# lyclyc52/Instance_NeRF

Measured on AMD Instinct MI355X. Metric: Msamples/sec (train+infer) 3D-FRONT 800x800 at 1/2/4/8 MI355X; PSNR parity, higher is better.
Workload: dtype f32; 1 GPU; render 800x800 synthetic 3D-FRONT-like room, hash-grid NeRF L=16 F=2 T=6119864 sigma+rgb (BASELINE configs[1]), one view per step per GPU; parallelism=views sharded over 1 GPU(s), no data-path collective

## Files before the change

### instance_nerf_amd/csrc/field_fused.hip

```cpp
#include <atomic>
#include <mutex>
#include <type_traits>

#include "common.h"
#include "grid_common.h"
#include "sample_pos.h"

namespace inr {

typedef float f32x4 __attribute__((ext_vector_type(4)));
typedef __bf16 bf16x8 __attribute__((ext_vector_type(8)));

#ifndef INR_MLP_FP32
#define INR_MLP_FP32 0
#endif

#ifdef INR_PROBE_BUILD
#include "probe/field_probe.h"
#else
#if defined(INR_PROBE_MODE) || defined(INR_PROBE_STATIC) || defined(INR_PROBE_SLOW_XCD)
#error "INR_PROBE_* switches need -DINR_PROBE_BUILD (tools/build_probe.py): those variants produce wrong results"
#endif
#define INR_PROBE_PROLOGUE()
#define INR_PROBE_SCHEDULE(steal)
// ... 362 lines not shown
__device__ __forceinline__ uint32_t pack_f16x2(float a, float b) {
  const f32x2_t v = {a, b};
  return __builtin_bit_cast(uint32_t, __builtin_convertvector(v, f16x2_t));
}
template <int N_MT, int N_S>
__device__ __forceinline__ void layer_h1(const uint4* __restrict__ w, int lane, const uint4* in, f32x4* out) {
  f32x4 acc[N_MT];
#pragma unroll
  for (int mt = 0; mt < N_MT; ++mt) acc[mt] = f32x4{0.f, 0.f, 0.f, 0.f};
#pragma unroll
  for (int st = 0; st < N_S; ++st) {
    __builtin_amdgcn_sched_barrier(0);
#pragma unroll
    for (int mt = 0; mt < N_MT; ++mt)
      acc[mt] = __builtin_amdgcn_mfma_f32_16x16x32_f16(__builtin_bit_cast(f16x8_t, w[((mt * N_S + st) * 2 + 0) * 64 + lane]),
                                                       __builtin_bit_cast(f16x8_t, in[st]), acc[mt], 0, 0, 0);
  }
#pragma unroll
  for (int mt = 0; mt < N_MT; ++mt) out[mt] = acc[mt];
}

template <int N_MT, int N_G, bool kFast = false>
__device__ __forceinline__ void mlp_layer(const float4* __restrict__ wsec, int lane, const f32x4* in, f32x4* out) {
#if INR_MLP_FP32
  layer<N_MT, N_G>(wsec, lane, in, out);
#else
  if constexpr (kFast) {
    uint4 b[N_G / 2];
#pragma unroll
    for (int st = 0; st < N_G / 2; ++st)
      b[st] = uint4{pack_f16x2(in[2 * st][0], in[2 * st][1]), pack_f16x2(in[2 * st][2], in[2 * st][3]),
                    pack_f16x2(in[2 * st + 1][0], in[2 * st + 1][1]), pack_f16x2(in[2 * st + 1][2], in[2 * st + 1][3])};
    layer_h1<N_MT, N_G / 2>(reinterpret_cast<const uint4*>(wsec), lane, b, out);
  } else {
    SplitB b[N_G / 2];
#pragma unroll
    for (int st = 0; st < N_G / 2; ++st) b[st] = split8(in[2 * st], in[2 * st + 1]);
    layer_bf<N_MT, N_G / 2>(reinterpret_cast<const uint4*>(wsec), lane, b, out);
  }
#endif
}

__device__ __forceinline__ float rgb_channel_of_lane(const f32x4 o) {
  const auto a = __builtin_amdgcn_permlane16_swap(__float_as_uint(o[0]), __float_as_uint(o[1]), false, false);
  const unsigned a0 = a[0];
  const auto b = __builtin_amdgcn_permlane32_swap(a0, __float_as_uint(o[2]), false, false);
  const unsigned b0 = b[0];
  return __uint_as_float(b0);
}
__device__ __forceinline__ float sigmoid_rgb(float o) {
  return __frcp_rn(1.0f + __expf(-o));
}

__device__ __forceinline__ float select4(int q, float a, float b, float c, float d) {
  return q == 0 ? a : (q == 1 ? b : (q == 2 ? c : d));
}

struct TileIn {
  float x0, x1, x2;
  float d0, d1, d2;
  bool oob;
};

__device__ __forceinline__ float to_x01(float x, float bound, float rb, float) { return (x + bound) / rb; }

template <bool kDir>
__device__ __forceinline__ void load_tile_in(const float* __restrict__ x, const float* __restrict__ d, int64_t m,
                                             float bound, float rb, float rb_inv, TileIn& t) {
  t.x0 = to_x01(x[m * 3 + 0], bound, rb, rb_inv);
  t.x1 = to_x01(x[m * 3 + 1], bound, rb, rb_inv);
  t.x2 = to_x01(x[m * 3 + 2], bound, rb, rb_inv);
  t.oob = oob01(t.x0, t.x1, t.x2);
  if (t.oob) t.x0 = t.x1 = t.x2 = 0.0f;
  if constexpr (kDir) {
    t.d0 = d[m * 3]; t.d1 = d[m * 3 + 1]; t.d2 = d[m * 3 + 2];
  }
}

constexpr int kXcdChunkLog2 = 10;
#ifndef INR_STEAL_SHIFT
#define INR_STEAL_SHIFT 1
#endif
constexpr int kStealRoundsShift = INR_STEAL_SHIFT;
struct TileSched {
  int64_t lo, hi;
  int64_t first;
  int64_t stride;
  int64_t main_local = 0, tail_base = 0;
  int64_t n_main = 0, tail = 0;
  int64_t static_local = 0;
  uint32_t xcd = 0;
  bool interleaved = false, hybrid = false;
  __device__ __forceinline__ int64_t tile_of(int y, int64_t u) const {
    if (u < main_local) return ((((u >> kXcdChunkLog2) << 3) + y) << kXcdChunkLog2) + (u & ((1 << kXcdChunkLog2) - 1));
    return n_main + tail * y / 8 + (u - main_local);
  }
  __device__ __forceinline__ int64_t local_end(int y) const { return main_local + tail * (y + 1) / 8 - tail * y / 8; }
  __device__ __forceinline__ int64_t tile(int64_t i) const {
    if (interleaved) {
      const int64_t u = first + i * stride;
      if (u < main_local)
        return ((((u >> kXcdChunkLog2) << 3) + xcd) << kXcdChunkLog2) + (u & ((1 << kXcdChunkLog2) - 1));
      return tail_base + (u - main_local);
    }
    return first + i * stride;
  }
};
__device__ __forceinline__ TileSched make_sched(int64_t n_tiles, int waves_per_block, bool steal = false) {
  const int nb = gridDim.x, b = blockIdx.x;
  const int w = threadIdx.x >> 6;
  TileSched s;
  if (nb % 8 == 0) {
    const int xcd = b & 7, local = b >> 3, per = nb >> 3;
    const int64_t rounds = n_tiles >> (kXcdChunkLog2 + 3);
    if (rounds >= 4) {
      const int64_t n_main = rounds << (kXcdChunkLog2 + 3), tail = n_tiles - n_main;
      s.interleaved = true;
      s.xcd = (uint32_t)xcd;
      s.main_local = rounds << kXcdChunkLog2;
      s.n_main = n_main;
      s.tail = tail;
      s.hybrid = steal;
      s.static_local = steal ? (rounds - max((int64_t)1, rounds >> kStealRoundsShift)) << kXcdChunkLog2 : s.main_local;
      s.tail_base = n_main + tail * xcd / 8;
      s.lo = 0;
      s.hi = n_main + tail * (xcd + 1) / 8;
      s.first = (int64_t)local * waves_per_block + w;
      s.stride = (int64_t)per * waves_per_block;
      return s;
    }
    s.lo = n_tiles * xcd / 8;
    s.hi = n_tiles * (xcd + 1) / 8;
    s.first = s.lo + (int64_t)local * waves_per_block + w;
    s.stride = (int64_t)per * waves_per_block;
  } else {
    s.lo = 0;
    s.hi = n_tiles;
    s.first = (int64_t)b * waves_per_block + w;
    s.stride = (int64_t)nb * waves_per_block;
  }
  return s;
}

constexpr int kFieldThreads = 512;
constexpr int kGroupChunkLog2 = 6;
constexpr int kGroupDraw = 1;
constexpr int kGroupPools = 4;
struct GroupDraw {
  unsigned long long* cursor;
  int owner, n_owner;
  __device__ __forceinline__ void init(unsigned long long* cursors, int pools) {
    const int n_xcd = (gridDim.x % 8 == 0) ? 8 : 1;
    const int n_pool = (gridDim.x % (8 * pools) == 0) ? pools : 1;
    const int xcd = (n_xcd == 8) ? (int)(blockIdx.x & 7) : 0;
    const int pool = (n_pool > 1) ? (int)((blockIdx.x >> 3) % pools) : 0;
    owner = pool * n_xcd + xcd;
    n_owner = n_pool * n_xcd;
    cursor = cursors + owner;
  }
  __device__ __forceinline__ int64_t group_of(uint32_t u) const {
    const int64_t chunk = (int64_t)(u >> kGroupChunkLog2) * n_owner + owner;
    return (chunk << kGroupChunkLog2) + (u & ((1u << kGroupChunkLog2) - 1u));
  }
  __device__ __forceinline__ int64_t draw() const { return group_of((uint32_t)atomicAdd(cursor, (unsigned long long)kGroupDraw)); }
};
constexpr int kStealPools = 4, kStealOwners = 8 * kStealPools, kStealDraw = 4, kStealBlockLog2 = 6;
struct TileWalk {
  TileSched s;
  unsigned long long* cur;
  int lane, own, owner, sub;
  int64_t it, k_base;
  unsigned long long raw_next;
  bool dyn;
  __device__ __forceinline__ void init(const TileSched& sched, unsigned long long* cursors) {
    s = sched; cur = cursors; lane = threadIdx.x & 63; it = 0; dyn = false; sub = kStealDraw; k_base = 0; raw_next = 0;
    own = owner = (int)(((blockIdx.x >> 3) % kStealPools) * 8 + (blockIdx.x & 7));
    if (!cursors) s.hybrid = false;
    if (!s.hybrid) s.static_local = s.main_local;
  }
  __device__ __forceinline__ int64_t pool_len(int o) const {
    const int64_t nb = (s.local_end(o & 7) - s.static_local + (1 << kStealBlockLog2) - 1) >> kStealBlockLog2;
    const int p = o >> 3;
    return nb > p ? ((nb - p + kStealPools - 1) / kStealPools) << kStealBlockLog2 : 0;
  }
  __device__ __forceinline__ int64_t local_of(int o, int64_t k) const {
    return s.static_local + ((((k >> kStealBlockLog2) * kStealPools) + (o >> 3)) << kStealBlockLog2) +
           (k & ((1 << kStealBlockLog2) - 1));
  }
  __device__ __forceinline__ unsigned long long issue(int o) const {
    unsigned long long v = 0;
    if (lane == 0) v = atomicAdd(cur + o, (unsigned long long)kStealDraw);
    return v;
  }
  __device__ __forceinline__ static int64_t uniform(unsigned long long v) {
    return (int64_t)(((unsigned long long)(uint32_t)__builtin_amdgcn_readfirstlane((int)(v >> 32)) << 32) |
                     (uint32_t)__builtin_amdgcn_readfirstlane((int)v));
  }
  __device__ __forceinline__ int scan() const {
    bool live = false;
    if (lane < kStealOwners) live = (int64_t)__hip_atomic_load(cur + lane, __ATOMIC_RELAXED, __HIP_MEMORY_SCOPE_AGENT) < pool_len(lane);
    const uint32_t mask = (uint32_t)__ballot(live);
    for (int i = 0; i < kStealOwners; ++i) {
      const int o = (((own >> 3) + i) % kStealPools) * 8 + (((own & 7) + i / kStealPools) & 7);
      if ((mask >> o) & 1u) return o;
    }
    return -1;
  }
  __device__ __forceinline__ int64_t next() {
    if (!dyn) {
      if (!s.hybrid) {
        const int64_t t = s.tile(it++);
        return t < s.hi ? t : -1;
      }
      const int64_t u = s.first + (it++) * s.stride;
      if (u < s.static_local) return s.tile_of((int)s.xcd, u);
      dyn = true;
      raw_next = issue(owner);
    }
    for (;;) {
      if (sub < kStealDraw) {
        const int64_t u = local_of(owner, k_base + sub);
        ++sub;
        if (u < s.local_end(owner & 7)) return s.tile_of(owner & 7, u);
        continue;
      }
      int64_t k = uniform(raw_next);
      while (k >= pool_len(owner)) {
        const int o = scan();
        if (o < 0) return -1;
        owner = o;
        k = uniform(issue(owner));
      }
      k_base = k;
      sub = 0;
      raw_next = issue(owner);
    }
  }
};
constexpr int kFieldMinWaves = 2;

__device__ __forceinline__ f32x4 load4(const float* p) {
  const float4 v = *reinterpret_cast<const float4*>(p);
  return f32x4{v.x, v.y, v.z, v.w};
}
__device__ __forceinline__ void store4(float* p, f32x4 v) {
  *reinterpret_cast<float4*>(p) = make_float4(v[0], v[1], v[2], v[3]);
}
__device__ __forceinline__ f32x4 mask4(f32x4 g, f32x4 h) {
  return f32x4{h[0] > 0.f ? g[0] : 0.f, h[1] > 0.f ? g[1] : 0.f, h[2] > 0.f ? g[2] : 0.f, h[3] > 0.f ? g[3] : 0.f};
}

struct NerfSave {
  float *enc, *h1, *so, *cin, *c1, *c2;
};

constexpr int kRayRowVec = INR_RAY_TABLE_FLOATS / 4;
template <bool kColor, bool kTable = false, int kSave = 0, bool kHalf = false, bool kFast = false, bool kPre = false,
          bool kRec = false>
__global__ void __launch_bounds__(kFieldThreads, kFieldMinWaves) k_nerf_fwd(const float* __restrict__ x, const float* __restrict__ d,
                                                               int64_t M, const int32_t* __restrict__ n_dev, float bound,
                                                               const float2* __restrict__ emb, uint32_t emb_bytes, GridDesc G,
                                                               const float4* __restrict__ packed, float density_scale,
                                                               float* __restrict__ sigma, float* __restrict__ rgb,
                                                               float* __restrict__ geo, const int32_t* __restrict__ ray_ids,
                                                               const float4* __restrict__ shq, NerfSave sv,
                                                               unsigned long long* __restrict__ steal) {
  extern __shared__ __attribute__((aligned(16))) float4 wl[];
  INR_PROBE_PROLOGUE();
  __builtin_amdgcn_s_setprio(3);
  constexpr int kStage = (kColor ? kNerfFloats : kCol0) / 4;
  for (int i = threadIdx.x; i < kStage; i += kFieldThreads) wl[i] = packed[i];
  LevelRec* recs = reinterpret_cast<LevelRec*>(wl + kStage);
  stage_level_recs(G, recs);
  __syncthreads();

  constexpr int kWaves = kFieldThreads / 64;
  const int lane = threadIdx.x & 63, q = lane >> 4, j = lane & 15;
  int64_t n = M;
  if (n_dev) n = min((int64_t)*n_dev, M);
  const int64_t n_tiles = (n + 15) >> 4;
  const float rb = 2.0f * bound;
  const float rb_inv = 0.0f;
  INR_PROBE_SCHEDULE(steal);
  TileWalk walk;
  walk.init(make_sched(n_tiles, kWaves, steal != nullptr), steal);

  const bool all_hashed[4] = {slot_all_hashed(G, 0), slot_all_hashed(G, 1), slot_all_hashed(G, 2), slot_all_hashed(G, 3)};
  const __amdgpu_buffer_rsrc_t rsrc = __builtin_amdgcn_make_buffer_rsrc((void*)emb, 0, (int)emb_bytes, 0x00020000);

  for (int64_t tile = walk.next(); tile >= 0; tile = walk.next()) {
    INR_PROBE_TILE();
    const int64_t m = tile * 16 + j;
    const bool valid = m < n;
    TileIn me;
    f32x4 sh_in = {0.f, 0.f, 0.f, 0.f};
    if constexpr (kRec) {
      static_assert(!kRec || (kTable && !kPre), "the records feed is a variant of the fused table feed");
      const int64_t mm = valid ? m : n - 1;
      const float t = x[mm];
      const float4* row = shq + (int64_t)ray_ids[mm] * kRayRowVec;
      const float4 t4 = row[q], o4 = row[4], d4 = row[5];
      sh_in = f32x4{t4.x, t4.y, t4.z, t4.w};
      const float rb_rcp = 1.0f / rb;
      me.x0 = sample_x01_pow2(sample_pos(o4.x, t, d4.x, bound), bound, rb_rcp);
      me.x1 = sample_x01_pow2(sample_pos(o4.y, t, d4.y, bound), bound, rb_rcp);
      me.x2 = sample_x01_pow2(sample_pos(o4.z, t, d4.z, bound), bound, rb_rcp);
    } else if constexpr (kTable) {
      const int64_t mm = valid ? m : n - 1;
      me.x0 = x[mm * 3 + 0]; me.x1 = x[mm * 3 + 1]; me.x2 = x[mm * 3 + 2];
      const float4 t4 = shq[(int64_t)ray_ids[mm] * 4 + q];
      sh_in = f32x4{t4.x, t4.y, t4.z, t4.w};
    } else {
      load_tile_in<kColor>(x, d, valid ? m : n - 1, bound, rb, rb_inv, me);
    }

    f32x4 enc[2];
    {
      Gathered g;
      uint32_t rec_off = (uint32_t)q * 4u * (uint32_t)sizeof(LevelRec);
      asm volatile("" : "+v"(rec_off));
      typedef float v2f __attribute__((ext_vector_type(2)));
// ... 9 lines not shown
      }
      issue_gathers<kHalf, kPre>(reinterpret_cast<const LevelRec*>(reinterpret_cast<const char*>(recs) + rec_off), all_hashed,
                                 rsrc, me.x0, me.x1, me.x2, g);
      __builtin_amdgcn_sched_barrier(0);
      blend<kHalf>(g, enc[0], enc[1]);
      if constexpr (kPre) {
        if (q == 2) enc[1] = f32x4{enc[1][0], enc[1][1], fine_a.x, fine_a.y};
        else if (q == 3) enc[1] = f32x4{fine_a.x, fine_a.y, fine_b.x, fine_b.y};
      }
    }
    if constexpr (!kTable) {
      if (me.oob) enc[0] = enc[1] = f32x4{0.f, 0.f, 0.f, 0.f};
    }
    INR_PROBE_AFTER_GATHER();

    f32x4 h1[4];
    mlp_layer<4, 2, kFast>(wl + kSig0 / 4, lane, enc, h1);
#pragma unroll
    for (int t = 0; t < 4; ++t) h1[t] = relu4(h1[t]);
    f32x4 h2[1];
    mlp_layer<1, 4, kFast>(wl + kSig1 / 4, lane, h1, h2);

    if (valid) {
      if (q == 0) sigma[m] = __expf(h2[0][0]) * density_scale;
      if (INR_PROBE_GEO_IS_OUTPUT && geo) {
#pragma unroll
        for (int r = 0; r < 4; ++r) {
          const int row = 4 * q + r;
          if (row >= 1) geo[m * 15 + row - 1] = h2[0][r];
        }
      }
    }

    if constexpr (kColor) {
      f32x4 cin[2];
      if constexpr (kTable) {
        cin[0] = sh_in;
      } else {
        float sh[16];
        sh4(me.d0, me.d1, me.d2, sh);
#pragma unroll
        for (int ks = 0; ks < 4; ++ks) cin[0][ks] = select4(q, sh[4 * ks], sh[4 * ks + 1], sh[4 * ks + 2], sh[4 * ks + 3]);
      }
      cin[1] = h2[0];
      f32x4 c1[4], c2[4], o[1];
      mlp_layer<4, 2, kFast>(wl + kCol0 / 4, lane, cin, c1);
#pragma unroll
      for (int t = 0; t < 4; ++t) c1[t] = relu4(c1[t]);
      mlp_layer<4, 4, kFast>(wl + kCol1 / 4, lane, c1, c2);
#pragma unroll
      for (int t = 0; t < 4; ++t) c2[t] = relu4(c2[t]);
      mlp_layer<1, 4, kFast>(wl + kCol2 / 4, lane, c2, o);
      if constexpr (kSave == 2) {
        if (valid) {
#pragma unroll
          for (int t = 0; t < 2; ++t) store4(sv.enc + m * 32 + 16 * t + 4 * q, enc[t]);
        }
      }
      if constexpr (kSave == 1) {
        if (valid) {
#pragma unroll
          for (int t = 0; t < 2; ++t) store4(sv.enc + m * 32 + 16 * t + 4 * q, enc[t]);
          store4(sv.so + m * 16 + 4 * q, h2[0]);
#pragma unroll
          for (int t = 0; t < 4; ++t) {
            store4(sv.h1 + m * 64 + 16 * t + 4 * q, h1[t]);
            store4(sv.c1 + m * 64 + 16 * t + 4 * q, c1[t]);
            store4(sv.c2 + m * 64 + 16 * t + 4 * q, c2[t]);
          }
#pragma unroll
          for (int ks = 0; ks < 4; ++ks) sv.cin[m * 32 + 4 * ks + q] = cin[0][ks];
#pragma unroll
          for (int r = 0; r < 4; ++r) {
            const int row = 4 * q + r;
            sv.cin[m * 32 + (row >= 1 ? 15 + row : 31)] = row >= 1 ? h2[0][r] : 0.f;
          }
        }
      }
      const float ch = sigmoid_rgb(rgb_channel_of_lane(o[0]));
      if (valid && q < 3) rgb[m * 3 + q] = ch;
    }
  }
  INR_PROBE_EPILOGUE();
}

constexpr int kSliceThreads = 256;
constexpr int kSliceTilesPerIter = 4;
struct SliceX {
  float x0, x1, x2;
};
__device__ __forceinline__ SliceX slice_load_x(const float* __restrict__ x01, int64_t m, int64_t M) {
  const int64_t mm = m < M ? m : M - 1;
  const float* p = x01 + mm * 3;
  return SliceX{__builtin_nontemporal_load(p), __builtin_nontemporal_load(p + 1), __builtin_nontemporal_load(p + 2)};
}
__global__ void __launch_bounds__(kSliceThreads) k_grid_fine_slices(const float* __restrict__ x01, int64_t M,
                                                                    const float2* __restrict__ emb, uint32_t emb_bytes,
                                                                    GridDesc G, float* __restrict__ pre) {
  const int slice = blockIdx.y;
  const int l = 16 - kSliceLevels + slice;
  const float sc = G.scales[l];
  const uint32_t m_ = G.mask[l], res1 = G.res1[l];
  const bool h = m_ != 0;
  const uint32_t base = G.offsets[l] * 8u, pa = h ? 2654435761u : res1, pb = h ? 805459861u : res1 * res1;
  const uint32_t mask = h ? m_ : 0xFFFFFFFFu;
  const __amdgpu_buffer_rsrc_t rsrc = __builtin_amdgcn_make_buffer_rsrc((void*)emb, 0, (int)emb_bytes, 0x00020000);
  const int lane = threadIdx.x & 63, w = threadIdx.x >> 6;
  const uint32_t side = (uint32_t)(lane & 1);
  constexpr int kWaves = kSliceThreads / 64;
  constexpr int kT = kSliceTilesPerIter;
  const int64_t m_pad = (M + 31) & ~(int64_t)31;
  const int64_t n_iter = (M + 32 * kT - 1) / (32 * kT);
  float* __restrict__ out = pre + (int64_t)slice * m_pad * 2;
  for (int64_t it = (int64_t)blockIdx.x * kWaves + w; it < n_iter; it += (int64_t)gridDim.x * kWaves) {
    u32x2 rows[kT][4];
    float wx[kT], fy[kT], fz[kT];
#pragma unroll
    for (int t = 0; t < kT; ++t) {
      const SliceX X = slice_load_x(x01, (it * kT + t) * 32 + (lane >> 1), M);
      const float px = X.x0 * sc + 0.5f, py = X.x1 * sc + 0.5f, pz = X.x2 * sc + 0.5f;
      const float fx = __builtin_amdgcn_fractf(px);
      wx[t] = side ? fx : 1.0f - fx;
      fy[t] = __builtin_amdgcn_fractf(py); fz[t] = __builtin_amdgcn_fractf(pz);
      const uint32_t c = (uint32_t)px + side, cy = (uint32_t)py, cz = (uint32_t)pz;
      const uint32_t hy0 = cy * pa, hy1 = hy0 + pa;
      const uint32_t hz0 = cz * pb, hz1 = hz0 + pb;
      const uint32_t yz[4] = {h ? (hy0 ^ hz0) : (hy0 + hz0), h ? (hy1 ^ hz0) : (hy1 + hz0),
                              h ? (hy0 ^ hz1) : (hy0 + hz1), h ? (hy1 ^ hz1) : (hy1 + hz1)};
#pragma unroll
      for (int k = 0; k < 4; ++k) {
        const uint32_t idx = (h ? (c ^ yz[k]) : (c + yz[k])) & mask;
        rows[t][k] = gather_row<false>(rsrc, base + idx * 8u);
      }
    }
#pragma unroll
    for (int t = 0; t < kT; ++t) {
      const f32x2 wy = {1.0f - fy[t], fy[t]};
      const f32x2 xy = wy * wx[t];
      const f32x2 w0 = xy * (1.0f - fz[t]), w1 = xy * fz[t];
      f32x2 acc = {0.f, 0.f};
      acc = __builtin_elementwise_fma(w0.xx, row2<false>(rows[t][0]), acc);
      acc = __builtin_elementwise_fma(w0.yy, row2<false>(rows[t][1]), acc);
      acc = __builtin_elementwise_fma(w1.xx, row2<false>(rows[t][2]), acc);
      acc = __builtin_elementwise_fma(w1.yy, row2<false>(rows[t][3]), acc);
      const float ox = __shfl_xor(acc.x, 1), oy = __shfl_xor(acc.y, 1);
      const float v = side ? acc.y + oy : acc.x + ox;
      const int64_t m = (it * kT + t) * 32 + (lane >> 1);
      if (m < M) __builtin_nontemporal_store(v, out + m * 2 + side);
    }
  }
}

struct LatticeDesc {
  const float* ax_w;
  const float* ax_l;
  const float* ax_h;
  int W, L, H, Wp;
};
constexpr int kMaxExtractDirs = 8;
template <bool kLattice>
__global__ void __launch_bounds__(kFieldThreads, kFieldMinWaves) k_nerf_fwd_dirs(
    const float* __restrict__ x, int64_t M, float bound, const float2* __restrict__ emb, uint32_t emb_bytes, GridDesc G,
    const float4* __restrict__ packed, const float* __restrict__ sh_dirs , int D, float4* __restrict__ out,
    LatticeDesc lat, float logit_min) {
  extern __shared__ __attribute__((aligned(16))) float4 wl[];
  constexpr int kStage = kNerfFloats / 4;
// ... 1417 lines not shown
};

struct FieldTable {
  GridDesc G;
  const float2* emb;
  uint32_t bytes;
};
static int field_table(const char* what, const inr_grid_desc* desc, const void* emb, bool half, FieldTable& t) {
  if (int rc = make_grid_desc(desc, t.G)) return rc;
  const uint64_t bytes = (uint64_t)desc->offsets[desc->num_levels] * (half ? 4ull : 8ull);
  if (bytes >= (1ull << 31)) {
    set_error("%s: table larger than 2 GiB is not addressable by the 32-bit gather offsets", what);
    return INR_EINVAL;
  }
  t.emb = reinterpret_cast<const float2*>(emb);
  t.bytes = (uint32_t)bytes;
  return INR_OK;
}
static const float4* f4(const float* p) { return reinterpret_cast<const float4*>(p); }

struct HybridSchedule {
  StealSet set;
  bool begin(hipStream_t s, int64_t n_tiles) {
    if ((n_tiles >> (kXcdChunkLog2 + 3)) < 4 || stream_is_capturing(s)) return true;
    set = steal_cursors(s);
    return set.cursors != nullptr;
  }
  unsigned long long* cursors() const { return set.cursors; }
  void finish(hipStream_t s) { steal_release(set, s); }
};

template <typename Kern, typename... Args>
static void launch_field(Kern kern, size_t lds, int64_t n_tiles, hipStream_t s, Args... args) {
  kern<<<grid_for(kern, lds, n_tiles), kFieldThreads, lds, s>>>(args...);
}

template <typename F>
static void with_kmt(int k_mt, F&& f) {
  switch (k_mt) {
    case 1: f(std::integral_constant<int, 1>{}); break;
    case 2: f(std::integral_constant<int, 2>{}); break;
    case 3: f(std::integral_constant<int, 3>{}); break;
    default: f(std::integral_constant<int, 4>{}); break;
  }
}
template <typename F>
static void with_flag(bool on, F&& f) {
  if (on) f(std::true_type{});
  else f(std::false_type{});
}
template <typename F>
static void with_mlp_f16(bool on, F&& f) {
#if !INR_MLP_FP32
  if (on) return f(std::true_type{});
#endif
  f(std::false_type{});
}

constexpr int kNumericsO = INR_NUMERICS_TABLE_F16 | INR_NUMERICS_MLP_F16;
constexpr unsigned kAcceptPlainOrO = 1u | 1u << kNumericsO;
constexpr unsigned kAcceptAny = 0xFu;
constexpr unsigned kAcceptPack = 1u | 1u << INR_NUMERICS_MLP_F16;
static int check_numerics(const char* what, int32_t numerics, unsigned accepted) {
  if (numerics < 0 || numerics > 3 || !((accepted >> numerics) & 1u)) {
    set_error("%s: numerics %d is not accepted here", what, numerics);
    return INR_EINVAL;
  }
#if INR_MLP_FP32
  if (numerics & INR_NUMERICS_MLP_F16) {
    set_error("%s: INR_NUMERICS_MLP_F16 is not available in the exact-fp32 build", what);
    return INR_EINVAL;
  }
#endif
  return INR_OK;
}

template <class KIdx>
static void pack_section_as(int32_t numerics, float* dst, const float* W, int n_out, int n_in, int n_mt, int n_ks,
                            KIdx kidx) {
  if (numerics & INR_NUMERICS_MLP_F16) pack_section_f16(dst, W, n_out, n_in, n_mt, n_ks, kidx);
  else pack_section(dst, W, n_out, n_in, n_mt, n_ks, kidx);
}

template <bool kRec>
static int forward_table_launch(const char* what, const float* x, const int32_t* ray_ids, const float* table, int64_t M,
                                float bound, const void* embeddings, const inr_grid_desc* desc, const float* packed,
                                float density_scale, float* sigma, float* rgb, int32_t numerics, inr_stream_t s) {
  FieldTable t;
  if (int rc = field_table(what, desc, embeddings, numerics & INR_NUMERICS_TABLE_F16, t)) return rc;
  if (int rc = check_numerics(what, numerics, kAcceptAny)) return rc;
  const size_t lds = std::max(kNerfFloats * sizeof(float) + kLevelRecBytes, (size_t)g_field_lds_min);
  const int64_t n_tiles = (M + 15) / 16;
  const hipStream_t st = as_stream(s);
  HybridSchedule hybrid;
  if (!hybrid.begin(st, n_tiles)) return INR_ELAUNCH;
  with_flag(numerics & INR_NUMERICS_TABLE_F16, [&](auto half) {
    with_mlp_f16(numerics & INR_NUMERICS_MLP_F16, [&](auto fast) {
      launch_field(k_nerf_fwd<true, true, 0, decltype(half)::value, decltype(fast)::value, false, kRec>, lds, n_tiles, st,
                   x, nullptr, M, nullptr, bound, t.emb, t.bytes, t.G, f4(packed), density_scale, sigma, rgb, nullptr,
                   ray_ids, f4(table), NerfSave{}, hybrid.cursors());
    });
  });
  hybrid.finish(st);
  return check_launch(what + 4);
}

__global__ void __launch_bounds__(256) k_ray_table_q(const float* __restrict__ o, const float* __restrict__ d, int64_t N,
                                                     float4* __restrict__ out) {
  const int64_t n = (int64_t)blockIdx.x * blockDim.x + threadIdx.x;
  if (n >= N) return;
  const float dx = d[n * 3], dy = d[n * 3 + 1], dz = d[n * 3 + 2];
  float v[16];
  sh4(dx, dy, dz, v);
  float4* row = out + n * kRayRowVec;
#pragma unroll
  for (int q = 0; q < 4; ++q) row[q] = make_float4(v[q], v[4 + q], v[8 + q], v[12 + q]);
  row[4] = make_float4(o[n * 3], o[n * 3 + 1], o[n * 3 + 2], 0.0f);
  row[5] = make_float4(dx, dy, dz, 0.0f);
}

}

using namespace inr;

extern "C" {

int64_t inr_nerf_packed_floats(void) { return kNerfFloats; }

int inr_nerf_pack_weights(const float* sigma_w0, const float* sigma_w1, const float* color_w0, const float* color_w1,
                          const float* color_w2, float* packed, int32_t numerics) {
  INR_REQUIRE(sigma_w0 && sigma_w1 && color_w0 && color_w1 && color_w2 && packed, "null pointer");
  if (int rc = check_numerics(__func__, numerics, kAcceptPack)) return rc;
  pack_section_as(numerics, packed + kSig0, sigma_w0, 64, 32, 4, 8, kidx_enc);
  pack_section_as(numerics, packed + kSig1, sigma_w1, 16, 64, 1, 16, kidx_hidden);
  pack_section_as(numerics, packed + kCol0, color_w0, 64, 31, 4, 8, kidx_color_in);
  pack_section_as(numerics, packed + kCol1, color_w1, 64, 64, 4, 16, kidx_hidden);
  pack_section_as(numerics, packed + kCol2, color_w2, 3, 64, 1, 16, kidx_hidden);
  return INR_OK;
}

int64_t inr_instance_packed_floats(int32_t K) {
  INR_REQUIRE(K > 0 && K <= 64 && K % 16 == 0, "K must be 16, 32, 48 or 64");
  return kIns2 + K * 64;
}

int inr_instance_pack_weights(const float* w0, const float* w1, const float* w2, int32_t K, float* packed,
                              int32_t numerics) {
  INR_REQUIRE(w0 && w1 && w2 && packed, "null pointer");
  INR_REQUIRE(K > 0 && K <= 64 && K % 16 == 0, "K must be 16, 32, 48 or 64");
  if (int rc = check_numerics(__func__, numerics, kAcceptPack)) return rc;
  pack_section_as(numerics, packed + kIns0, w0, 64, 32, 4, 8, kidx_enc);
  pack_section_as(numerics, packed + kIns1, w1, 64, 64, 4, 16, kidx_hidden);
  pack_section_as(numerics, packed + kIns2, w2, K, 64, K / 16, 16, kidx_hidden);
  return INR_OK;
}

int inr_nerf_forward(const float* x, const float* d, int64_t M, const int32_t* n_samples_dev, float bound,
                     const void* embeddings, const inr_grid_desc* desc, const float* packed, float density_scale,
                     float* sigma, float* rgb, float* geo_feat, int32_t numerics, inr_stream_t s) {
  const bool o = numerics == kNumericsO;
  INR_REQUIRE(M >= 0 && desc, "bad argument");
  if (M == 0) return INR_OK;
  INR_REQUIRE(x && embeddings && packed && sigma && (rgb || !o), "null pointer");
  INR_REQUIRE(!rgb || d, "rgb requested without view directions");
  INR_REQUIRE(!(o && geo_feat), "no geo_feat under the -O numerics");
  INR_REQUIRE(((uintptr_t)embeddings & (o ? 3 : 7)) == 0 && ((uintptr_t)packed & 15) == 0, "embeddings/packed misaligned");
  FieldTable t;
  if (int rc = field_table(__func__, desc, embeddings, o, t)) return rc;
  if (int rc = check_numerics(__func__, numerics, kAcceptPlainOrO)) return rc;
  const int64_t n_tiles = (M + 15) / 16;
  const hipStream_t st = as_stream(s);
  HybridSchedule hybrid;
  if (!o && !hybrid.begin(st, n_tiles)) return INR_ELAUNCH;
  const size_t lds = (rgb ? kNerfFloats : kCol0) * sizeof(float) + kLevelRecBytes;
  const auto launch = [&](auto kern) {
    launch_field(kern, lds, n_tiles, st, x, d, M, n_samples_dev, bound, t.emb, t.bytes, t.G, f4(packed), density_scale,
                 sigma, rgb, geo_feat, nullptr, nullptr, NerfSave{}, hybrid.cursors());
  };
// ... 455 lines not shown
```

Before: 6632 Msamples/s.

## Add paired-tile forward field kernel splitting hash-grid gathers across half-waves

Adds k_nerf_fwd_pair, which processes two 16-sample tiles per wave iteration. Each half of the wave gathers coarse levels for one tile and one x-side of the fine-level corners for both tiles, then exchanges partial encodings with permlane swaps before running the MLP per tile. The aim is to increase memory-level parallelism and cut redundant per-tile gather work, with explicit vmcnt waits interleaving the coarse and fine loads. The tile scheduler and stealer are templated on a unit shift so they walk pairs instead of tiles. The new path is used for the recorded-table forward when all fine levels are hashed and default numerics are in effect, with an env var to disable it; it adds complexity and register pressure.

Measured after the change: 7225 Msamples/s, median of 6. 8.9% higher.

```diff
diff --git a/instance_nerf_amd/csrc/field_fused.hip b/instance_nerf_amd/csrc/field_fused.hip
--- a/instance_nerf_amd/csrc/field_fused.hip
+++ b/instance_nerf_amd/csrc/field_fused.hip
@@ -468,7 +468,9 @@
 #define INR_STEAL_SHIFT 1
 #endif
 constexpr int kStealRoundsShift = INR_STEAL_SHIFT;
-struct TileSched {
+template <int kUnit = 0>
+struct TileSchedT {
+  static constexpr int kChunkLog2 = kXcdChunkLog2 - kUnit;
   int64_t lo, hi;
   int64_t first;
   int64_t stride;
@@ -478,7 +480,7 @@
   uint32_t xcd = 0;
   bool interleaved = false, hybrid = false;
   __device__ __forceinline__ int64_t tile_of(int y, int64_t u) const {
-    if (u < main_local) return ((((u >> kXcdChunkLog2) << 3) + y) << kXcdChunkLog2) + (u & ((1 << kXcdChunkLog2) - 1));
+    if (u < main_local) return ((((u >> kChunkLog2) << 3) + y) << kChunkLog2) + (u & ((1 << kChunkLog2) - 1));
     return n_main + tail * y / 8 + (u - main_local);
   }
   __device__ __forceinline__ int64_t local_end(int y) const { return main_local + tail * (y + 1) / 8 - tail * y / 8; }
@@ -486,28 +488,31 @@
     if (interleaved) {
       const int64_t u = first + i * stride;
       if (u < main_local)
-        return ((((u >> kXcdChunkLog2) << 3) + xcd) << kXcdChunkLog2) + (u & ((1 << kXcdChunkLog2) - 1));
+        return ((((u >> kChunkLog2) << 3) + xcd) << kChunkLog2) + (u & ((1 << kChunkLog2) - 1));
       return tail_base + (u - main_local);
     }
     return first + i * stride;
   }
 };
-__device__ __forceinline__ TileSched make_sched(int64_t n_tiles, int waves_per_block, bool steal = false) {
+using TileSched = TileSchedT<>;
+template <int kUnit = 0>
+__device__ __forceinline__ TileSchedT<kUnit> make_sched(int64_t n_tiles, int waves_per_block, bool steal = false) {
+  constexpr int kChunkLog2 = TileSchedT<kUnit>::kChunkLog2;
   const int nb = gridDim.x, b = blockIdx.x;
   const int w = threadIdx.x >> 6;
-  TileSched s;
+  TileSchedT<kUnit> s;
   if (nb % 8 == 0) {
     const int xcd = b & 7, local = b >> 3, per = nb >> 3;
-    const int64_t rounds = n_tiles >> (kXcdChunkLog2 + 3);
+    const int64_t rounds = n_tiles >> (kChunkLog2 + 3);
     if (rounds >= 4) {
-      const int64_t n_main = rounds << (kXcdChunkLog2 + 3), tail = n_tiles - n_main;
+      const int64_t n_main = rounds << (kChunkLog2 + 3), tail = n_tiles - n_main;
       s.interleaved = true;
       s.xcd = (uint32_t)xcd;
-      s.main_local = rounds << kXcdChunkLog2;
+      s.main_local = rounds << kChunkLog2;
       s.n_main = n_main;
       s.tail = tail;
       s.hybrid = steal;
-      s.static_local = steal ? (rounds - max((int64_t)1, rounds >> kStealRoundsShift)) << kXcdChunkLog2 : s.main_local;
+      s.static_local = steal ? (rounds - max((int64_t)1, rounds >> kStealRoundsShift)) << kChunkLog2 : s.main_local;
       s.tail_base = n_main + tail * xcd / 8;
       s.lo = 0;
       s.hi = n_main + tail * (xcd + 1) / 8;
@@ -551,31 +556,33 @@
   __device__ __forceinline__ int64_t draw() const { return group_of((uint32_t)atomicAdd(cursor, (unsigned long long)kGroupDraw)); }
 };
 constexpr int kStealPools = 4, kStealOwners = 8 * kStealPools, kStealDraw = 4, kStealBlockLog2 = 6;
-struct TileWalk {
-  TileSched s;
+template <int kUnit = 0>
+struct TileWalkT {
+  static constexpr int kBlockLog2 = kStealBlockLog2 - kUnit, kDraw = kStealDraw >> kUnit;
+  TileSchedT<kUnit> s;
   unsigned long long* cur;
   int lane, own, owner, sub;
   int64_t it, k_base;
   unsigned long long raw_next;
   bool dyn;
-  __device__ __forceinline__ void init(const TileSched& sched, unsigned long long* cursors) {
-    s = sched; cur = cursors; lane = threadIdx.x & 63; it = 0; dyn = false; sub = kStealDraw; k_base = 0; raw_next = 0;
+  __device__ __forceinline__ void init(const TileSchedT<kUnit>& sched, unsigned long long* cursors) {
+    s = sched; cur = cursors; lane = threadIdx.x & 63; it = 0; dyn = false; sub = kDraw; k_base = 0; raw_next = 0;
     own = owner = (int)(((blockIdx.x >> 3) % kStealPools) * 8 + (blockIdx.x & 7));
     if (!cursors) s.hybrid = false;
     if (!s.hybrid) s.static_local = s.main_local;
   }
   __device__ __forceinline__ int64_t pool_len(int o) const {
-    const int64_t nb = (s.local_end(o & 7) - s.static_local + (1 << kStealBlockLog2) - 1) >> kStealBlockLog2;
+    const int64_t nb = (s.local_end(o & 7) - s.static_local + (1 << kBlockLog2) - 1) >> kBlockLog2;
     const int p = o >> 3;
-    return nb > p ? ((nb - p + kStealPools - 1) / kStealPools) << kStealBlockLog2 : 0;
+    return nb > p ? ((nb - p + kStealPools - 1) / kStealPools) << kBlockLog2 : 0;
   }
   __device__ __forceinline__ int64_t local_of(int o, int64_t k) const {
-    return s.static_local + ((((k >> kStealBlockLog2) * kStealPools) + (o >> 3)) << kStealBlockLog2) +
-           (k & ((1 << kStealBlockLog2) - 1));
+    return s.static_local + ((((k >> kBlockLog2) * kStealPools) + (o >> 3)) << kBlockLog2) +
+           (k & ((1 << kBlockLog2) - 1));
   }
   __device__ __forceinline__ unsigned long long issue(int o) const {
     unsigned long long v = 0;
-    if (lane == 0) v = atomicAdd(cur + o, (unsigned long long)kStealDraw);
+    if (lane == 0) v = atomicAdd(cur + o, (unsigned long long)kDraw);
     return v;
   }
   __device__ __forceinline__ static int64_t uniform(unsigned long long v) {
@@ -604,7 +611,7 @@
       raw_next = issue(owner);
     }
     for (;;) {
-      if (sub < kStealDraw) {
+      if (sub < kDraw) {
         const int64_t u = local_of(owner, k_base + sub);
         ++sub;
         if (u < s.local_end(owner & 7)) return s.tile_of(owner & 7, u);
@@ -623,6 +630,7 @@
     }
   }
 };
+using TileWalk = TileWalkT<>;
 constexpr int kFieldMinWaves = 2;
 
 __device__ __forceinline__ f32x4 load4(const float* p) {
@@ -798,6 +806,212 @@
     }
   }
   INR_PROBE_EPILOGUE();
+}
+
+#ifndef INR_PAIR_WAIT_COARSE
+#define INR_PAIR_WAIT_COARSE 16
+#endif
+#ifndef INR_PAIR_WAIT_FINE
+#define INR_PAIR_WAIT_FINE 8
+#endif
+constexpr int kPairWaitAfterCoarse = INR_PAIR_WAIT_COARSE;
+constexpr int kPairWaitBetweenFine = INR_PAIR_WAIT_FINE;
+struct GatheredPair {
+  u32x2 c[4][8];
+  u32x2 f[8][4];
+  float cfx[4], cfy[4], cfz[4];
+  float fwx[8], ffy[8], ffz[8];
+};
+
+__device__ __forceinline__ void issue_coarse_pair(const LevelRec* __restrict__ my_recs, __amdgpu_buffer_rsrc_t rsrc, float x0,
+                                                  float x1, float x2, GatheredPair& g) {
+#pragma unroll
+  for (int c = 0; c < 4; ++c) {
+    const LevelRec* rec = my_recs + (c >> 1) * 8 + (c & 1);
+    const uint4 ra = rec->a;
+    const float s = __uint_as_float(ra.x);
+    const uint32_t base = ra.y, pa = ra.z, pb = ra.w;
+    const uint4 rb = rec->b;
+    const uint32_t mask = rb.x;
+    const float px = x0 * s + 0.5f, py = x1 * s + 0.5f, pz = x2 * s + 0.5f;
+    g.cfx[c] = __builtin_amdgcn_fractf(px); g.cfy[c] = __builtin_amdgcn_fractf(py); g.cfz[c] = __builtin_amdgcn_fractf(pz);
+    const uint32_t cx = (uint32_t)px, cy = (uint32_t)py, cz = (uint32_t)pz;
+    const uint32_t hy0 = cy * pa, hy1 = hy0 + pa;
+    const uint32_t hz0 = cz * pb, hz1 = hz0 + pb;
+    const IndexTerms t = index_terms(hy0, hy1, hz0, hz1, rb.z, rb.w);
+    uint32_t off[8];
+#pragma unroll
+    for (int k = 0; k < 8; ++k) off[k] = base + t.row(cx + (k & 1), k >> 1, mask) * 8u;
+#pragma unroll
+    for (int k = 0; k < 8; ++k) g.c[c][k] = gather_at(rsrc, off[k]);
+    keep_offsets(off[0], off[1], off[2], off[3]);
+    keep_offsets(off[4], off[5], off[6], off[7]);
+  }
+}
+
+template <int kFirst>
+__device__ __forceinline__ void issue_fine_pair(const GridDesc& G, __amdgpu_buffer_rsrc_t rsrc, uint32_t side, float x0, float x1,
+                                                float x2, GatheredPair& g) {
+#pragma unroll
+  for (int i = kFirst; i < kFirst + 4; ++i) {
+    const float s = G.scales[8 + i];
+    const uint32_t base = G.offsets[8 + i] * 8u, mask = G.mask[8 + i];
+    const uint32_t pa = 2654435761u, pb = 805459861u;
+    const float px = x0 * s + 0.5f, py = x1 * s + 0.5f, pz = x2 * s + 0.5f;
+    const float fx = __builtin_amdgcn_fractf(px);
+    g.fwx[i] = side ? fx : 1.0f - fx;
+    g.ffy[i] = __builtin_amdgcn_fractf(py); g.ffz[i] = __builtin_amdgcn_fractf(pz);
+    const uint32_t c = (uint32_t)px + side, cy = (uint32_t)py, cz = (uint32_t)pz;
+    const uint32_t hy0 = cy * pa, hy1 = hy0 + pa;
+    const uint32_t hz0 = cz * pb, hz1 = hz0 + pb;
+    if (i == 0) wait_vmcnt<kPairWaitAfterCoarse>();
+    else wait_vmcnt<kPairWaitBetweenFine>();
+    uint32_t off[4];
+    off[0] = base + ((c ^ (hy0 ^ hz0)) & mask) * 8u;
+    off[1] = base + ((c ^ (hy1 ^ hz0)) & mask) * 8u;
+    off[2] = base + ((c ^ (hy0 ^ hz1)) & mask) * 8u;
+    off[3] = base + ((c ^ (hy1 ^ hz1)) & mask) * 8u;
+#pragma unroll
+    for (int k = 0; k < 4; ++k) g.f[i][k] = gather_at(rsrc, off[k]);
+    keep_offsets(off[0], off[1], off[2], off[3]);
+  }
+}
+
+__device__ __forceinline__ void blend_coarse_pair(const GatheredPair& g, f32x4 (&p)[2], f32x4 (&r)[2]) {
+#pragma unroll
+  for (int c = 0; c < 4; ++c) {
+    const f32x2 wx = {1.0f - g.cfx[c], g.cfx[c]};
+    const float wy0 = 1.0f - g.cfy[c], wz0 = 1.0f - g.cfz[c];
+    const f32x2 a = wx * wy0, b = wx * g.cfy[c];
+    const f32x2 w[4] = {a * wz0, b * wz0, a * g.cfz[c], b * g.cfz[c]};
+    f32x2 acc = {0.f, 0.f};
+#pragma unroll
+    for (int k = 0; k < 8; ++k) {
+      const f32x2 wk = (k & 1) ? w[k >> 1].yy : w[k >> 1].xx;
+      acc = __builtin_elementwise_fma(wk, row2(g.c[c][k]), acc);
+    }
+    f32x4& out = (c >> 1) ? r[0] : p[0];
+    out[2 * (c & 1)] = acc.x;
+    out[2 * (c & 1) + 1] = acc.y;
+  }
+}
+__device__ __forceinline__ void blend_fine_pair(const GatheredPair& g, f32x4 (&p)[2], f32x4 (&r)[2]) {
+  f32x2 part[8];
+#pragma unroll
+  for (int i = 0; i < 8; ++i) {
+    const f32x2 wy = {1.0f - g.ffy[i], g.ffy[i]};
+    const f32x2 xy = wy * g.fwx[i];
+    const f32x2 w0 = xy * (1.0f - g.ffz[i]), w1 = xy * g.ffz[i];
+    f32x2 acc = {0.f, 0.f};
+    acc = __builtin_elementwise_fma(w0.xx, row2(g.f[i][0]), acc);
+    acc = __builtin_elementwise_fma(w0.yy, row2(g.f[i][1]), acc);
+    acc = __builtin_elementwise_fma(w1.xx, row2(g.f[i][2]), acc);
+    acc = __builtin_elementwise_fma(w1.yy, row2(g.f[i][3]), acc);
+    part[i] = acc;
+  }
+#pragma unroll
+  for (int k = 0; k < 4; ++k) {
+    const int i0 = (k >> 1) * 4 + (k & 1);
+#pragma unroll
+    for (int ft = 0; ft < 2; ++ft) {
+      const auto v = __builtin_amdgcn_permlane16_swap(__float_as_uint(part[i0][ft]), __float_as_uint(part[i0 + 2][ft]), false, false);
+      const unsigned v0 = v[0], v1 = v[1];
+      f32x4& out = (k >> 1) ? r[1] : p[1];
+      out[2 * (k & 1) + ft] = __uint_as_float(v0) + __uint_as_float(v1);
+    }
+  }
+}
+
+__device__ __forceinline__ void pair_tile_mlp(const float4* __restrict__ wl, int lane, bool valid, int64_t m, const f32x4 (&enc)[2],
+                                              f32x4 sh_in, float density_scale, float* __restrict__ sigma,
+                                              float* __restrict__ rgb) {
+  const int q = lane >> 4;
+  f32x4 h1[4];
+  mlp_layer<4, 2>(wl + kSig0 / 4, lane, enc, h1);
+#pragma unroll
+  for (int t = 0; t < 4; ++t) h1[t] = relu4(h1[t]);
+  f32x4 h2[1];
+  mlp_layer<1, 4>(wl + kSig1 / 4, lane, h1, h2);
+  if (valid && q == 0) sigma[m] = __expf(h2[0][0]) * density_scale;
+  f32x4 cin[2] = {sh_in, h2[0]};
+  f32x4 c1[4], c2[4], o[1];
+  mlp_layer<4, 2>(wl + kCol0 / 4, lane, cin, c1);
+#pragma unroll
+  for (int t = 0; t < 4; ++t) c1[t] = relu4(c1[t]);
+  mlp_layer<4, 4>(wl + kCol1 / 4, lane, c1, c2);
+#pragma unroll
+  for (int t = 0; t < 4; ++t) c2[t] = relu4(c2[t]);
+  mlp_layer<1, 4>(wl + kCol2 / 4, lane, c2, o);
+  const float ch = sigmoid_rgb(rgb_channel_of_lane(o[0]));
+  if (valid && q < 3) rgb[m * 3 + q] = ch;
+}
+
+__global__ void __launch_bounds__(kFieldThreads, kFieldMinWaves) k_nerf_fwd_pair(
+    const float* __restrict__ x, int64_t M, float bound, const float2* __restrict__ emb, uint32_t emb_bytes, GridDesc G,
+    const float4* __restrict__ packed, float density_scale, float* __restrict__ sigma, float* __restrict__ rgb,
+    const int32_t* __restrict__ ray_ids, const float4* __restrict__ shq, unsigned long long* __restrict__ steal) {
+  extern __shared__ __attribute__((aligned(16))) float4 wl[];
+  __builtin_amdgcn_s_setprio(3);
+  constexpr int kStage = kNerfFloats / 4;
+  for (int i = threadIdx.x; i < kStage; i += kFieldThreads) wl[i] = packed[i];
+  LevelRec* recs = reinterpret_cast<LevelRec*>(wl + kStage);
+  stage_level_recs(G, recs);
+  __syncthreads();
+
+  constexpr int kWaves = kFieldThreads / 64;
+  const int lane = threadIdx.x & 63, q = lane >> 4, j = lane & 15, h = lane >> 5;
+  const uint32_t side = (uint32_t)(q & 1);
+  const int64_t n = M;
+  const int64_t n_tiles = (n + 15) >> 4, n_pairs = (n_tiles + 1) >> 1;
+  const float rb_rcp = 1.0f / (2.0f * bound);
+  TileWalkT<1> walk;
+  walk.init(make_sched<1>(n_pairs, kWaves, steal != nullptr), steal);
+  const __amdgpu_buffer_rsrc_t rsrc = __builtin_amdgcn_make_buffer_rsrc((void*)emb, 0, (int)emb_bytes, 0x00020000);
+
+  for (int64_t pair = walk.next(); pair >= 0; pair = walk.next()) {
+    const int64_t mg = pair * 32 + h * 16 + j;
+    const int64_t mm = mg < n ? mg : n - 1;
+    const float t = x[mm];
+    const int32_t rid = ray_ids[mm];
+    const float4* row = shq + (int64_t)rid * kRayRowVec;
+    const float4 o4 = row[4], d4 = row[5];
+    const auto rr = __builtin_amdgcn_permlane32_swap((unsigned)rid, (unsigned)rid, false, false);
+    const unsigned rid_a = rr[0], rid_b = rr[1];
+    const float4 sa = shq[(int64_t)(int32_t)rid_a * kRayRowVec + q], sb = shq[(int64_t)(int32_t)rid_b * kRayRowVec + q];
+    const float x0 = sample_x01_pow2(sample_pos(o4.x, t, d4.x, bound), bound, rb_rcp);
+    const float x1 = sample_x01_pow2(sample_pos(o4.y, t, d4.y, bound), bound, rb_rcp);
+    const float x2 = sample_x01_pow2(sample_pos(o4.z, t, d4.z, bound), bound, rb_rcp);
+
+    f32x4 enc_a[2], enc_b[2];
+    {
+      GatheredPair g;
+      uint32_t rec_off = side * 4u * (uint32_t)sizeof(LevelRec);
+      asm volatile("" : "+v"(rec_off));
+      issue_coarse_pair(reinterpret_cast<const LevelRec*>(reinterpret_cast<const char*>(recs) + rec_off), rsrc, x0, x1, x2, g);
+      issue_fine_pair<0>(G, rsrc, side, x0, x1, x2, g);
+      __builtin_amdgcn_sched_barrier(0);
+      blend_coarse_pair(g, enc_a, enc_b);
+      __builtin_amdgcn_sched_barrier(0);
+      issue_fine_pair<4>(G, rsrc, side, x0, x1, x2, g);
+      __builtin_amdgcn_sched_barrier(0);
+      blend_fine_pair(g, enc_a, enc_b);
+    }
+#pragma unroll
+    for (int e = 0; e < 2; ++e) {
+#pragma unroll
+      for (int c = 0; c < 4; ++c) {
+        const auto v = __builtin_amdgcn_permlane32_swap(__float_as_uint(enc_a[e][c]), __float_as_uint(enc_b[e][c]), false, false);
+        const unsigned v0 = v[0], v1 = v[1];
+        enc_a[e][c] = __uint_as_float(v0);
+        enc_b[e][c] = __uint_as_float(v1);
+      }
+    }
+
+    const int64_t ma = pair * 32 + j, mb = ma + 16;
+    pair_tile_mlp(wl, lane, ma < n, ma, enc_a, f32x4{sa.x, sa.y, sa.z, sa.w}, density_scale, sigma, rgb);
+    if (pair * 2 + 1 < n_tiles)
+      pair_tile_mlp(wl, lane, mb < n, mb, enc_b, f32x4{sb.x, sb.y, sb.z, sb.w}, density_scale, sigma, rgb);
+  }
 }
 
 constexpr int kSliceThreads = 256;
@@ -2381,6 +2595,17 @@
   else pack_section(dst, W, n_out, n_in, n_mt, n_ks, kidx);
 }
 
+static bool pair_front_end_qualifies(const inr_grid_desc* desc, int32_t numerics) {
+#if INR_MLP_FP32
+  return false;
+#endif
+  if (numerics != 0 || desc->num_levels != 16) return false;
+  for (int l = 8; l < 16; ++l)
+    if (!desc->hashed[l]) return false;
+  const char* off = getenv("INR_FIELD_PAIR");
+  return !(off && off[0] == '0' && off[1] == 0);
+}
+
 template <bool kRec>
 static int forward_table_launch(const char* what, const float* x, const int32_t* ray_ids, const float* table, int64_t M,
                                 float bound, const void* embeddings, const inr_grid_desc* desc, const float* packed,
@@ -2393,6 +2618,12 @@
   const hipStream_t st = as_stream(s);
   HybridSchedule hybrid;
   if (!hybrid.begin(st, n_tiles)) return INR_ELAUNCH;
+  if (kRec && pair_front_end_qualifies(desc, numerics)) {
+    launch_field(k_nerf_fwd_pair, lds, (n_tiles + 1) / 2, st, x, M, bound, t.emb, t.bytes, t.G, f4(packed), density_scale,
+                 sigma, rgb, ray_ids, f4(table), hybrid.cursors());
+    hybrid.finish(st);
+    return check_launch(what + 4);
+  }
   with_flag(numerics & INR_NUMERICS_TABLE_F16, [&](auto half) {
     with_mlp_f16(numerics & INR_NUMERICS_MLP_F16, [&](auto fast) {
       launch_field(k_nerf_fwd<true, true, 0, decltype(half)::value, decltype(fast)::value, false, kRec>, lds, n_tiles, st,
```
